# uniio/ivf-hnsw

Hardware: AMD Instinct MI355X
Metric: queries/sec @ Recall@1, SIFT1B PQ16 nprobe=32; ADC scan HBM GB/s vs peak (higher is better)
Workload: dtype f32

## Files before the change

ivf-hnsw_amd/csrc/capi_handle.cpp:

```cpp
#include "capi_internal.h"

#include <cstdarg>

static thread_local std::string g_last_error;

namespace ivfhnsw_gpu_impl {

int fail(int code, const char *fmt, ...)
{
    char buf[512];
    va_list ap;
    va_start(ap, fmt);
    vsnprintf(buf, sizeof(buf), fmt, ap);
    va_end(ap);
    g_last_error = buf;
    return code;
}

int bind(ivfhnsw_gpu *h)
{
    if (!h)
        return fail(IVFHNSW_ERR_INVALID, "null handle");
    HIP_TRY(hipSetDevice(h->device));
    return IVFHNSW_OK;
// ... 18 lines not shown
    }
    hipEvent_t e = nullptr;
    (void)hipEventCreate(&e);
    return e;
}

int drain_events(ivfhnsw_gpu *h)
{
    for (auto &ev : h->pending) {
        HIP_TRY(hipEventSynchronize(ev.b));
        float ms = 0.f;
        HIP_TRY(hipEventElapsedTime(&ms, ev.a, ev.b));
        h->stage_ms[ev.stage] += ms;
        h->stage_n[ev.stage] += 1;
        h->pool.push_back(ev.a);
        h->pool.push_back(ev.b);
    }
    h->pending.clear();
    return IVFHNSW_OK;
}

int check_status(ivfhnsw_gpu *h)
{
    uint32_t st = 0;
    HIP_TRY(hipMemcpy(&st, &status_words(h)->bits, sizeof(st), hipMemcpyDeviceToHost));
    if (!st)
        return IVFHNSW_OK;
    HIP_TRY(hipMemset(&status_words(h)->bits, 0, sizeof(st)));
    if (st & kStatusHnswTieOverflow)
        return fail(IVFHNSW_ERR_STATE, "HNSW walk: more than 64 candidates tie exactly with the efSearch-th "
                                       "distance; results of this batch are invalid");
    if (st & kStatusTopkStreamOverflow)
        return fail(IVFHNSW_ERR_STATE, "heap-order top-k: candidate stream of a query exceeded %u entries; use "
                                       "heap_order = 0 for this k / max_codes", kHeapStreamCap);
    return fail(IVFHNSW_ERR_STATE, "device status 0x%x", st);
}

void follow_parent(ivfhnsw_gpu *view, const ivfhnsw_gpu *parent)
{
    view->t = parent->t;
    view->has_ivf = parent->has_ivf;
    view->n_local = parent->n_local;
    view->g = parent->g;
    view->has_group = parent->has_group;
    view->gr = parent->gr;
    view->has_graph = parent->has_graph;
    view->filter_mode = parent->filter_mode;
    view->fmask = parent->fmask;
    view->f_pass = parent->f_pass;
}

int table_change_guard(ivfhnsw_gpu *h, TableChange what, const char *who, bool need_ivf)
{
    if (h && h->is_view) {
        static const char *const kinds[] = {"uploads", "appends", "removals"};
        return fail(IVFHNSW_ERR_STATE, "%s%s%s go to the handle that holds the tables, not to a view of it",
                    what == kUploads ? "" : who, what == kUploads ? "" : ": ", kinds[what]);
    }
    int rc = bind(h);
    if (rc)
        return rc;
    if (need_ivf && !h->has_ivf)
        return fail(IVFHNSW_ERR_STATE, "%s before upload_ivf", who);
    return IVFHNSW_OK;
}

void point_at_lists(ivfhnsw_gpu *h, uint64_t n_local)
{
    h->t.goff = h->goff.as<uint64_t>();
    h->t.loff = h->loff.as<uint32_t>();
    h->t.codes = h->codes.as<uint8_t>();
    h->t.norm_codes = h->ncodes.as<uint8_t>();
    h->t.ids = h->ids.as<uint32_t>();
    h->n_local = n_local;
}

}

const char *ivfhnsw_gpu_last_error(void) { return g_last_error.c_str(); }

int ivfhnsw_gpu_abi_version(void) { return 9; }

int ivfhnsw_gpu_device_count(int *count)
{
    if (!count)
        return fail(IVFHNSW_ERR_INVALID, "null argument");
    int n = 0;
    hipError_t e = hipGetDeviceCount(&n);
    if (e != hipSuccess)
        return fail(IVFHNSW_ERR_HIP, "hipGetDeviceCount: %s", hipGetErrorString(e));
    *count = n;
    return IVFHNSW_OK;
}

static int split_permille_env()
{
    static const int v = [] {
        const char *e = getenv("IVFHNSW_SPLIT");
        const int x = (e && *e) ? atoi(e) : kSplitAuto;
        return (x > 0 && x <= kSplitAuto) ? x : 0;
    }();
    return v;
}

int ivfhnsw_gpu_create(int device, ivfhnsw_gpu **out)
{
    if (!out)
        return fail(IVFHNSW_ERR_INVALID, "null out pointer");
    *out = nullptr;
    int ndev = 0;
    hipError_t e = hipGetDeviceCount(&ndev);
    if (e != hipSuccess || ndev == 0)
        return fail(IVFHNSW_ERR_HIP, "no HIP device available (%s); there is no CPU fallback",
                    e == hipSuccess ? "device count 0" : hipGetErrorString(e));
    if (device < 0 || device >= ndev)
        return fail(IVFHNSW_ERR_INVALID, "device %d out of range (have %d)", device, ndev);
    HIP_TRY(hipSetDevice(device));
    hipDeviceProp_t prop;
    HIP_TRY(hipGetDeviceProperties(&prop, device));
    if (strncmp(prop.gcnArchName, "gfx950", 6) != 0)
        return fail(IVFHNSW_ERR_HIP, "device %d is %s; this library holds gfx950 code only", device, prop.gcnArchName);
    ivfhnsw_gpu *h = new ivfhnsw_gpu();
    h->device = device;
    hipError_t se = hipStreamCreateWithFlags(&h->stream, hipStreamNonBlocking);
    if (se != hipSuccess) {
        delete h;
        return fail(IVFHNSW_ERR_HIP, "hipStreamCreate: %s", hipGetErrorString(se));
    }
    h->own_stream = true;
    h->split_pm = split_permille_env();
    if (h->w_status.ensure(sizeof(StatusWords)) || hipMemset(h->w_status.p, 0, sizeof(StatusWords)) != hipSuccess) {
        ivfhnsw_gpu_destroy(h);
        return fail(IVFHNSW_ERR_HIP, "cannot allocate the device status word");
    }
    *out = h;
    return IVFHNSW_OK;
}

int ivfhnsw_gpu_destroy(ivfhnsw_gpu *h)
{
    if (!h)
        return IVFHNSW_OK;
    (void)hipSetDevice(h->device);
    (void)hipStreamSynchronize(h->stream);
    if (h->split_view) {
        ivfhnsw_gpu_destroy(h->split_view);
        h->split_view = nullptr;
        (void)hipSetDevice(h->device);
    }
    if (h->split_fork)
        (void)hipEventDestroy(h->split_fork);
    if (h->split_join)
        (void)hipEventDestroy(h->split_join);
    for (auto &ev : h->pending) {
        (void)hipEventDestroy(ev.a);
        (void)hipEventDestroy(ev.b);
    }
    for (auto e : h->pool)
        (void)hipEventDestroy(e);
    h->for_each_devbuf([](DevBuf &b) { b.release(); });
    h->p_in.release();
    h->p_out.release();
    if (h->own_stream)
        (void)hipStreamDestroy(h->stream);
    delete h;
    return IVFHNSW_OK;
}

int ivfhnsw_gpu_create_view(ivfhnsw_gpu *parent, ivfhnsw_gpu **out)
{
    if (!out)
        return fail(IVFHNSW_ERR_INVALID, "null out pointer");
    *out = nullptr;
    int rc = bind(parent);
    if (rc)
        return rc;
    if (parent->is_view)
        return fail(IVFHNSW_ERR_INVALID, "a view of a view: create it from the handle that holds the tables");
    HIP_TRY(hipStreamSynchronize(parent->stream));
    ivfhnsw_gpu *h = nullptr;
    if ((rc = ivfhnsw_gpu_create(parent->device, &h)))
        return rc;
    h->is_view = true;
    h->split_pm = 0;
    follow_parent(h, parent);
    h->parent = parent;
    *out = h;
    return IVFHNSW_OK;
}

int ivfhnsw_gpu_set_stream(ivfhnsw_gpu *h, void *hip_stream)
{
    int rc = bind(h);
    if (rc)
        return rc;
    HIP_TRY(hipStreamSynchronize(h->stream));
    if (h->own_stream)
        (void)hipStreamDestroy(h->stream);
    h->stream = reinterpret_cast<hipStream_t>(hip_stream);
    h->own_stream = false;
    return IVFHNSW_OK;
}

int ivfhnsw_gpu_sync(ivfhnsw_gpu *h)
{
    int rc = bind(h);
    if (rc)
        return rc;
    HIP_TRY(hipStreamSynchronize(h->stream));
    return check_status(h);
}

int ivfhnsw_gpu_set_batch_split(ivfhnsw_gpu *h, int permille)
{
    if (!h)
        return fail(IVFHNSW_ERR_INVALID, "null handle");
    if (permille < 0 || permille > kSplitAuto)
        return fail(IVFHNSW_ERR_INVALID, "batch split %d outside 0..999 permille (1000 = by estimate)", permille);
    if (h->is_view && permille)
        return fail(IVFHNSW_ERR_INVALID, "a view cannot split its batches (it is what the second part runs on)");
    h->split_pm = permille;
    return IVFHNSW_OK;
}

int ivfhnsw_gpu_set_option(ivfhnsw_gpu *h, const char *key, long value)
{
    if (!h || !key)
        return fail(IVFHNSW_ERR_INVALID, "set_option: null argument");
    if (!strcmp(key, "scan_pipe")) {
        if (value < -1 || value > 1)
            return fail(IVFHNSW_ERR_INVALID, "set_option scan_pipe: %ld outside -1..1", value);
        h->opt_scan_pipe = (int)value;
        return IVFHNSW_OK;
    }
    if (!strcmp(key, "exact_splits")) {
        if (value != -1 && (value < 1 || value > 64))
            return fail(IVFHNSW_ERR_INVALID, "set_option exact_splits: %ld is neither -1 nor in 1..64", value);
        h->opt_exact_splits = (int)value;
        return IVFHNSW_OK;
    }
    return fail(IVFHNSW_ERR_INVALID, "set_option: unknown key '%s'", key);
}

int ivfhnsw_gpu_set_profiling(ivfhnsw_gpu *h, int enabled)
{
    int rc = bind(h);
    if (rc)
        return rc;
    h->profiling = enabled == 2 ? 2 : (enabled != 0 ? 1 : 0);
    if (h->split_view)
        h->split_view->profiling = h->profiling;
    return IVFHNSW_OK;
}

int ivfhnsw_gpu_get_stage_ms(ivfhnsw_gpu *h, int stage, double *ms_total, uint64_t *launches)
{
    int rc = bind(h);
    if (rc)
        return rc;
    if (stage < 0 || stage >= IVFHNSW_STAGE_COUNT)
        return fail(IVFHNSW_ERR_INVALID, "bad stage %d", stage);
    if ((rc = drain_events(h)))
        return rc;
    double ms = h->stage_ms[stage];
    uint64_t n = h->stage_n[stage];
    if (h->split_view) {
        if ((rc = drain_events(h->split_view)))
            return rc;
        ms += h->split_view->stage_ms[stage];
        n += h->split_view->stage_n[stage];
    }
    if (ms_total)
        *ms_total = ms;
    if (launches)
        *launches = n;
    return IVFHNSW_OK;
}

int ivfhnsw_gpu_reset_stage_ms(ivfhnsw_gpu *h)
{
    int rc = bind(h);
    if (rc)
        return rc;
    if ((rc = drain_events(h)))
        return rc;
    for (int i = 0; i < IVFHNSW_STAGE_COUNT; i++) {
        h->stage_ms[i] = 0;
        h->stage_n[i] = 0;
    }
    if (h->split_view)
        return ivfhnsw_gpu_reset_stage_ms(h->split_view);
    return IVFHNSW_OK;
}

int ivfhnsw_gpu_last_scan_counts(ivfhnsw_gpu *h, uint64_t *ncodes, uint64_t *nsegments)
{
    int rc = bind(h);
    if (rc)
        return rc;
    unsigned long long out[2] = {0, 0};
    if (h->last_nq) {
        HIP_TRY(launch_plan_totals(h->stream, h->w_hdr.as<PlanHdr>(), h->last_nq,
                                   h->w_totals.as<unsigned long long>()));
        HIP_TRY(hipMemcpyAsync(out, h->w_totals.p, sizeof(out), hipMemcpyDeviceToHost, h->stream));
        HIP_TRY(hipStreamSynchronize(h->stream));
    }
// ... 38 lines not shown
```

ivf-hnsw_amd/csrc/capi_internal.h:

```cpp
#pragma once
#include "../../include/ivfhnsw_hip.h"
#include "ivfhnsw_kernels.h"

#include <hip/hip_runtime.h>

#include <algorithm>
#include <new>
#include <cmath>
#include <cstddef>
#include <cstdio>
#include <cstdlib>
#include <cstring>
#include <string>
#include <unordered_map>
#include <vector>

namespace ivfhnsw_gpu_impl {

int fail(int code, const char *fmt, ...) __attribute__((format(printf, 2, 3)));

#define HIP_TRY(expr)                                                                                        \
    do {                                                                                                     \
        hipError_t e_ = (expr);                                                                              \
        if (e_ != hipSuccess)                                                                                \
            return fail(e_ == hipErrorOutOfMemory ? IVFHNSW_ERR_NOMEM : IVFHNSW_ERR_HIP, "%s: %s (%s:%d)",   \
                        #expr, hipGetErrorString(e_), __FILE__, __LINE__);                                   \
    } while (0)

struct DevBuf {
    void *p = nullptr;
    size_t bytes = 0;
    int ensure(size_t need)
    {
        if (need <= bytes)
            return IVFHNSW_OK;
        release();
        HIP_TRY(hipMalloc(&p, need ? need : 1));
        bytes = need;
        return IVFHNSW_OK;
    }
    void release()
    {
        if (p)
            (void)hipFree(p);
        p = nullptr;
        bytes = 0;
    }
    template <class T> T *as() const { return reinterpret_cast<T *>(p); }
};

struct HostBuf {
    void *p = nullptr;
    size_t bytes = 0;
    int ensure(size_t need)
    {
        if (need <= bytes)
            return IVFHNSW_OK;
        release();
        HIP_TRY(hipHostMalloc(&p, need ? need : 1, hipHostMallocDefault));
        bytes = need;
        return IVFHNSW_OK;
    }
    void release()
    {
        if (p)
            (void)hipHostFree(p);
        p = nullptr;
        bytes = 0;
    }
    template <class T> T *as() const { return reinterpret_cast<T *>(p); }
};

struct StageEvent {
    int stage;
    hipEvent_t a, b;
};

struct StatusWords {
    uint32_t bits;
    uint32_t walk_next;
    uint32_t redo_len;
    uint32_t redo_next;
    uint32_t redo_exits;
    uint32_t heap_redo_len;
    uint32_t heap_redo_exits;
    uint32_t pad;
};
static_assert(offsetof(StatusWords, redo_len) == offsetof(StatusWords, walk_next) + 4 &&
                  offsetof(StatusWords, redo_next) == offsetof(StatusWords, walk_next) + 8 &&
                  offsetof(StatusWords, redo_exits) == offsetof(StatusWords, walk_next) + 12,
              "launch_coarse: next_query is followed by the three words of the redo header");
static_assert(offsetof(StatusWords, heap_redo_exits) == offsetof(StatusWords, heap_redo_len) + 4, "launch_heap_scan: redo_hdr[0..1]");
static_assert(offsetof(StatusWords, bits) == 0 && sizeof(StatusWords) == 8 * sizeof(uint32_t), "8 words, bits first");

struct WalkScratch {
    bool zero = false;
    void *zero_ptr = nullptr;
    size_t zero_bytes = 0;
    bool counters_clean = true;
};

}

using namespace ivfhnsw_gpu_impl;

#define IVFHNSW_GPU_DEVBUFS(X) \
    X(goff) X(loff) X(cnorm) X(pqc) X(ntab) X(opq_at) X(codes) X(ncodes) X(ids)  \
    X(g_alpha) X(g_nn) X(g_sizes) X(g_inter)  \
    X(q_counts) X(q_links) X(q_vectors) X(q_qrows) X(q_nbrows) X(q_nbnorms) X(q_fat) X(q_links_c)  \
    X(e_pqc) X(e_ntab) X(e_a) X(e_at) X(e_x) X(e_idx) X(e_dist) X(e_res) X(e_tmp) X(e_codes) X(e_ncodes)  \
    X(t_x) X(t_y) X(t_cb) X(t_assign) X(t_part) X(t_c)  \
    X(k_q) X(k_x) X(k_qn) X(k_xn) X(k_part) X(k_ids) X(k_dists)  \
    X(km_x) X(km_c) X(km_assign) X(km_dist) X(km_cnt) X(km_start) X(km_ids) X(km_ids2) X(km_hist) X(km_part) X(km_status) X(km_pairs)  \
    X(gb_table) X(gb_fwd) X(gb_fcnt) X(gb_deg) X(gb_roff) X(gb_ids) X(gb_ids2) X(gb_hist) X(gb_stat) X(gb_counts) X(gb_links)  \
    X(cg_q) X(cg_cidx) X(cg_ids) X(cg_dists) X(gc_nn) X(cg_cvn) X(cg_tab) X(cg_tab2) X(cg_off) X(cg_alpha2) X(cg_sub)  \
    X(base_rows) X(base_stage)  \
    X(r_q) X(r_cand) X(r_dist) X(r_lab)  \
    X(ex_q) X(ex_part) X(ex_raw) X(ex_dist) X(ex_lab)  \
    X(ap_idx) X(ap_ids) X(ap_codes) X(ap_ncodes) X(ap_cnt) X(ap_own) X(ap_part) X(ap_status) X(ap_perm) X(ap_perm2) X(ap_hist) X(ap_tiles)  \
    X(gp_sub) X(gp_sizes) X(gp_pre_old) X(gp_pre_new) X(gp_rows) X(gp_gather) X(ga_cidx) X(ga_off) X(ga_nn) X(ga_alpha) X(ga_inter) X(ga_status)  \
    X(rm_labels) X(rm_bits) X(rm_mask) X(rm_keep) X(rm_rem) X(rm_out) X(rm_part) X(rm_status) X(rm_sizes)  \
    X(f_mask) X(f_bits) X(f_labels) X(f_count)  \
    X(w_xq) X(w_luts) X(w_segs) X(w_lpos) X(w_hdr) X(w_keys) X(w_cid) X(w_cd) X(w_qsd) X(w_totals) X(w_visited) X(w_status) X(w_stream) X(w_slen) X(w_tail) X(w_redo) X(w_hredo) X(w_heap)  \
    X(rg_dist) X(rg_lab) X(rg_slices) X(rg_part) X(rg_lims)  \
    X(s_q) X(s_cid) X(s_cd) X(s_dist) X(s_lab) X(s_keys) X(s_len)

struct ivfhnsw_gpu {
    int device = 0;
    hipStream_t stream = nullptr;
    bool own_stream = false;
    bool is_view = false;

#define IVFHNSW_X(name) DevBuf name;
    IVFHNSW_GPU_DEVBUFS(IVFHNSW_X)
#undef IVFHNSW_X
    template <class F> void for_each_devbuf(F &&f)
    {
#define IVFHNSW_X(name) f(name);
        IVFHNSW_GPU_DEVBUFS(IVFHNSW_X)
#undef IVFHNSW_X
    }
    HostBuf p_in, p_out;

    IvfTables t{};
    bool has_ivf = false;
    uint64_t n_local = 0;
    GroupTables g{};
    bool has_group = false;
    GraphTables gr{};
    bool has_graph = false;
    size_t e_d = 0, e_M = 0;
    bool e_opq = false, has_codebooks = false;
    uint64_t base_n = 0;
    size_t base_d = 0;
    ivfhnsw_gpu *parent = nullptr;

    int filter_mode = -1;
    const uint32_t *fmask = nullptr;
    bool f_has_bits = false;
    uint32_t f_max_label = 0;
    uint64_t f_pass = 0;

    ivfhnsw_gpu *split_view = nullptr;
    hipEvent_t split_fork = nullptr, split_join = nullptr;
    bool last_split = false;
    uint32_t *status_shared = nullptr;
    size_t last_parts[2] = {0, 0};
    int split_pm = 0;
    WalkScratch walk;
    int opt_scan_pipe = -1;
    int opt_exact_splits = -1;

    int last_nq = 0, last_max_seg = 0;
    const char *last_scan_kernel = "";
    bool last_stream = false;
    bool last_range = false;

    bool rg_valid = false;
    uint64_t rg_total = 0;

    int profiling = 0;
    std::vector<StageEvent> pending;
    std::vector<hipEvent_t> pool;
    double stage_ms[IVFHNSW_STAGE_COUNT] = {0};
    uint64_t stage_n[IVFHNSW_STAGE_COUNT] = {0};
};

namespace ivfhnsw_gpu_impl {

int bind(ivfhnsw_gpu *h);
int upload(DevBuf &b, const void *src, size_t bytes);
hipEvent_t take_event(ivfhnsw_gpu *h);
int drain_events(ivfhnsw_gpu *h);
int check_status(ivfhnsw_gpu *h);

inline StatusWords *status_words(ivfhnsw_gpu *h) { return h->w_status.as<StatusWords>(); }
inline uint32_t *status_word(ivfhnsw_gpu *h) { return h->status_shared ? h->status_shared : &status_words(h)->bits; }

void follow_parent(ivfhnsw_gpu *view, const ivfhnsw_gpu *parent);

enum TableChange { kUploads, kAppends, kRemovals };
int table_change_guard(ivfhnsw_gpu *h, TableChange what, const char *who, bool need_ivf);

void point_at_lists(ivfhnsw_gpu *h, uint64_t n_local);

int filter_mark_rows(ivfhnsw_gpu *h, const uint32_t *ids, uint64_t n_local, DevBuf &mask, uint64_t *pass);
void filter_drop(ivfhnsw_gpu *h);

struct ListArrays {
    DevBuf goff, loff, codes, ncodes, ids;
    DevBuf fmask;
    uint64_t fpass = 0;
    ListArrays() = default;
    ListArrays(const ListArrays &) = delete;
    ListArrays &operator=(const ListArrays &) = delete;
    ~ListArrays() { release(); }
    int allocate(size_t nc, uint64_t n_local, size_t M)
    {
        int rc;
        if ((rc = goff.ensure((nc + 1) * sizeof(uint64_t))) || (rc = loff.ensure(nc * sizeof(uint32_t))) ||
            (rc = codes.ensure(n_local * M)) || (rc = ncodes.ensure(n_local)) || (rc = ids.ensure(n_local * sizeof(uint32_t))))
            return rc;
        return IVFHNSW_OK;
    }
    int mark_filter(ivfhnsw_gpu *h, uint64_t n_local)
    {
        if (h->filter_mode < 0)
            return IVFHNSW_OK;
        return filter_mark_rows(h, ids.as<uint32_t>(), n_local, fmask, &fpass);
    }
    void release()
    {
        for (DevBuf *b : {&goff, &loff, &codes, &ncodes, &ids, &fmask})
            b->release();
    }
    void install(ivfhnsw_gpu *h, uint64_t n_local)
    {
        if (h->filter_mode >= 0) {
            std::swap(h->f_mask, fmask);
            h->fmask = h->f_mask.as<uint32_t>();
            h->f_pass = fpass;
        }
        std::swap(h->goff, goff);
        std::swap(h->loff, loff);
        std::swap(h->codes, codes);
        std::swap(h->ncodes, ncodes);
        std::swap(h->ids, ids);
        release();
        point_at_lists(h, n_local);
    }
};

struct StageScope {
    ivfhnsw_gpu *h;
    StageEvent ev{};
    bool on;
    StageScope(ivfhnsw_gpu *h_, int stage)
        : h(h_), on(h_->profiling == 1 || (h_->profiling == 2 && stage == IVFHNSW_STAGE_SCAN))
    {
        if (!on)
            return;
        ev.stage = stage;
        ev.a = take_event(h);
        ev.b = take_event(h);
        (void)hipEventRecord(ev.a, h->stream);
    }
    ~StageScope()
    {
        if (!on)
            return;
        (void)hipEventRecord(ev.b, h->stream);
        h->pending.push_back(ev);
    }
};

constexpr uint32_t kHeapStreamCap = 8192;

constexpr int kSplitAuto = 1000;

constexpr size_t kMaxBatchAll = 1 << 17;

struct SearchCall {
    uint32_t *status_out = nullptr;
    bool defer_redo = false;
    bool no_latency = false;
    bool wrote_status = false;
};

struct WalkClear {
    uint64_t *keys = nullptr;
    uint32_t *done = nullptr;
    bool cleared = false;
};

struct SearchArgs {
    size_t nq, k;
    const float *d_queries;
    const uint32_t *d_coarse_ids;
    const float *d_coarse_dists;
    const ivfhnsw_search_params *p;
    float *d_distances;
    int64_t *d_labels, *d_out_keys;
    SearchArgs slice(size_t q0, size_t n, size_t d) const
    {
        return {n, k, d_queries + q0 * d, d_coarse_ids ? d_coarse_ids + q0 * p->nprobe : nullptr,
                d_coarse_dists ? d_coarse_dists + q0 * p->nprobe : nullptr, p, d_distances + q0 * k, d_labels + q0 * k,
                d_out_keys};
    }
};

struct Chunk : SearchArgs {
    int nprobe, max_seg, plan_k;
    bool heap_big;
    const uint32_t *fmask;
    const float *xq;
    const uint32_t *cid;
    const float *cd;
    bool use_tail;
    WalkClear meet;
    int nsplit;
    bool heap, pipe;
};

int search_args_guard(const ivfhnsw_gpu *h, const ivfhnsw_search_params *p, size_t k);
int stage_in(ivfhnsw_gpu *h, DevBuf &b, const void *src, size_t bytes);
int stage_out(ivfhnsw_gpu *h, void *dst, const DevBuf &b, size_t bytes);
int chunk_checks(ivfhnsw_gpu *h, const Chunk &c, bool results = true);
int chunk_workspace(ivfhnsw_gpu *h, Chunk &c);
int chunk_coarse(ivfhnsw_gpu *h, Chunk &c, const SearchCall &call);
int chunk_plan_table(ivfhnsw_gpu *h, Chunk &c);

void range_drop(ivfhnsw_gpu *h);

int grouping_dedupe_reserve(ivfhnsw_gpu *h);
int grouping_dedupe_dev(ivfhnsw_gpu *h, const uint32_t *d_sizes, const uint32_t *d_nn, int *dedupe);

int encode_rows(ivfhnsw_gpu *h, size_t m, float *dx, const float *table, const uint32_t *rows);
int encode_groups_impl(ivfhnsw_gpu *h, size_t ngroups, size_t nsubc, const uint32_t *centroid_idx,
                       const uint64_t *offsets, const float *x, size_t efSearch, uint32_t *out_nn_centroid_idxs,
                       float *out_alphas, uint32_t *out_subcentroid_idxs, uint8_t *out_codes, uint8_t *out_norm_codes,
                       bool dev, bool stage);

}
```

ivf-hnsw_amd/csrc/capi_search.cpp:

```cpp
#include "capi_internal.h"

static size_t env_size(const char *name, size_t def)
{
    const char *e = getenv(name);
    return (e && *e) ? (size_t)atol(e) : def;
}

int ivfhnsw_gpu_impl::search_args_guard(const ivfhnsw_gpu *h, const ivfhnsw_search_params *p, size_t k)
{
    if (!h->has_ivf)
        return fail(IVFHNSW_ERR_STATE, "search before upload_ivf");
    if (!p || p->nprobe == 0 || k == 0)
        return fail(IVFHNSW_ERR_INVALID, "nprobe and k must be positive");
    return IVFHNSW_OK;
}

int ivfhnsw_gpu_impl::stage_in(ivfhnsw_gpu *h, DevBuf &b, const void *src, size_t bytes)
{
    int rc = b.ensure(bytes);
    if (rc)
        return rc;
    HIP_TRY(hipMemcpyAsync(b.p, src, bytes, hipMemcpyHostToDevice, h->stream));
    return IVFHNSW_OK;
}

int ivfhnsw_gpu_impl::stage_out(ivfhnsw_gpu *h, void *dst, const DevBuf &b, size_t bytes)
{
    HIP_TRY(hipMemcpyAsync(dst, b.p, bytes, hipMemcpyDeviceToHost, h->stream));
    return IVFHNSW_OK;
}

static int walk_scratch(ivfhnsw_gpu *h, size_t words, size_t nslots, size_t nq, uint32_t **tails)
{
    int rc = h->w_visited.ensure(words * sizeof(uint32_t) * std::max<size_t>(nslots, 64) * 2);
    if (rc)
        return rc;
    if (h->w_visited.p != h->walk.zero_ptr || h->w_visited.bytes != h->walk.zero_bytes) {
        HIP_TRY(hipMemsetAsync(h->w_visited.p, 0, h->w_visited.bytes, h->stream));
        h->walk.zero = true;
        h->walk.zero_ptr = h->w_visited.p;
        h->walk.zero_bytes = h->w_visited.bytes;
    }
    *tails = reinterpret_cast<uint32_t *>(h->w_visited.as<char>() + h->w_visited.bytes / 2);
    return h->w_redo.ensure(nq * sizeof(uint32_t));
}

static int coarse_dev_impl(ivfhnsw_gpu *h, size_t nq, const float *d_queries, size_t nprobe, size_t efSearch,
                           uint32_t *d_coarse_ids, float *d_coarse_dists, const SearchCall &call, WalkClear &meet)
{
    int rc = bind(h);
    if (rc)
        return rc;
    if (!h->has_graph)
        return fail(IVFHNSW_ERR_STATE, "coarse search needs upload_quantizer");
    if (nprobe == 0 || efSearch < nprobe)
        return fail(IVFHNSW_ERR_INVALID, "efSearch %zu < nprobe %zu (precondition of IndexIVF_HNSW.cpp:249-258)",
                    efSearch, nprobe);
    if (efSearch > 1024)
        return fail(IVFHNSW_ERR_INVALID, "efSearch %zu > 1024 unsupported on the device", efSearch);
    if (nq == 0)
        return IVFHNSW_OK;
    if (nq > 0x7fffffffull)
        return fail(IVFHNSW_ERR_INVALID, "nq too large");
    const size_t words = ((((size_t)h->gr.n + 31) / 32) + 3) & ~(size_t)3;
    StageScope sc(h, IVFHNSW_STAGE_COARSE);
    static const size_t lat_max_nq = env_size("IVFHNSW_LATENCY_MAX_NQ", 256);
    StatusWords *st = status_words(h);
    uint32_t *tails = nullptr;
    if (!call.no_latency && nq <= lat_max_nq && coarse_latency_supported(h->gr, (int)efSearch)) {
        uint32_t *hdr = &st->redo_len;
        const bool defer = call.defer_redo;
        if (!defer) {
            if ((rc = walk_scratch(h, words, 64, nq, &tails)))
                return rc;
            HIP_TRY(hipMemsetAsync(hdr, 0, 3 * sizeof(uint32_t), h->stream));
        }
        HIP_TRY(launch_coarse_latency(h->stream, h->gr, d_queries, (int)nq, (int)nprobe, (int)efSearch, d_coarse_ids,
                                      d_coarse_dists, status_word(h), meet.keys, meet.done, defer ? nullptr : hdr,
                                      defer ? nullptr : h->w_redo.as<uint32_t>()));
        meet.cleared = meet.keys != nullptr;
        if (!defer)
            HIP_TRY(launch_coarse_redo(h->stream, h->gr, d_queries, (int)nq, (int)nprobe, (int)efSearch, d_coarse_ids,
                                       d_coarse_dists, h->w_visited.as<uint32_t>(), words, status_word(h), hdr,
                                       h->w_redo.as<uint32_t>(), tails, 64));
        return IVFHNSW_OK;
    }
    const int nslots = (int)std::min<size_t>(nq, (size_t)coarse_slots_for((int)efSearch));
    if ((rc = walk_scratch(h, words, (size_t)nslots, nq, &tails)))
        return rc;
    HIP_TRY(launch_coarse(h->stream, h->gr, d_queries, (int)nq, (int)nprobe, (int)efSearch, d_coarse_ids, d_coarse_dists,
                          h->w_visited.as<uint32_t>(), words, nslots, status_word(h), &st->walk_next,
                          h->w_visited.bytes / 2, &h->walk.zero, h->w_redo.as<uint32_t>(), tails, 64,
                          &h->walk.counters_clean));
    return IVFHNSW_OK;
}

int ivfhnsw_gpu_coarse_dev(ivfhnsw_gpu *h, size_t nq, const float *d_queries, size_t nprobe, size_t efSearch,
                           uint32_t *d_coarse_ids, float *d_coarse_dists)
{
    WalkClear meet;
    return coarse_dev_impl(h, nq, d_queries, nprobe, efSearch, d_coarse_ids, d_coarse_dists, SearchCall(), meet);
}

int ivfhnsw_gpu_rotate_dev(ivfhnsw_gpu *h, size_t nq, const float *d_queries, float *d_out)
{
    int rc = bind(h);
    if (rc)
        return rc;
    if (!h->has_ivf)
        return fail(IVFHNSW_ERR_STATE, "rotate needs upload_ivf");
    if (nq == 0)
        return IVFHNSW_OK;
    if (!d_queries || !d_out || nq > 0x7fffffffull)
        return fail(IVFHNSW_ERR_INVALID, "null buffer or nq too large");
    if (h->t.opq_At) {
        StageScope sc(h, IVFHNSW_STAGE_OPQ);
        HIP_TRY(launch_opq(h->stream, h->t.opq_At, d_queries, d_out, (int)nq, h->t.d));
    } else if (d_out != d_queries) {
        HIP_TRY(hipMemcpyAsync(d_out, d_queries, nq * (size_t)h->t.d * sizeof(float), hipMemcpyDeviceToDevice, h->stream));
    }
    return IVFHNSW_OK;
}

int ivfhnsw_gpu_coarse(ivfhnsw_gpu *h, size_t nq, const float *queries, size_t k, size_t efSearch, uint32_t *ids,
                       float *dists)
{
    int rc = bind(h);
    if (rc)
        return rc;
    if (!h->has_graph)
        return fail(IVFHNSW_ERR_STATE, "coarse search needs upload_quantizer");
    if (nq == 0)
        return IVFHNSW_OK;
    if (!queries || !ids || !dists || k == 0)
        return fail(IVFHNSW_ERR_INVALID, "null buffer or k == 0");
    const size_t d = h->gr.d;
    if ((rc = h->s_cid.ensure(nq * k * sizeof(uint32_t))) || (rc = h->s_cd.ensure(nq * k * sizeof(float))) ||
        (rc = stage_in(h, h->s_q, queries, nq * d * sizeof(float))) ||
        (rc = ivfhnsw_gpu_coarse_dev(h, nq, h->s_q.as<float>(), k, efSearch, h->s_cid.as<uint32_t>(), h->s_cd.as<float>())) ||
        (rc = stage_out(h, ids, h->s_cid, nq * k * sizeof(uint32_t))) ||
        (rc = stage_out(h, dists, h->s_cd, nq * k * sizeof(float))))
        return rc;
    HIP_TRY(hipStreamSynchronize(h->stream));
    return check_status(h);
}

static int search_dev_chunk(ivfhnsw_gpu *h, const SearchArgs &a, SearchCall &call);

static const size_t kSplitMinNq = 8192;

static int auto_split_permille(const ivfhnsw_gpu *h, const ivfhnsw_search_params *p)
{
    const double walk = 1.7 * (double)p->efSearch;
    const double nc = (double)std::max<uint32_t>(h->t.nc, 1u);
    const double list = (double)h->n_local / nc;
    const double codes = std::min((double)p->nprobe * list, (double)p->max_codes + 0.5 * list);
    double scan = codes * (double)(h->t.M + 1) / 5000.0 + 5.0;
    if (h->has_group)
        scan = scan / 0.8 + 90.0;
    const double share = walk / (walk + scan);
    return (int)std::min(900.0, std::max(400.0, share * 1000.0 + 0.5));
}

static int search_dev_split(ivfhnsw_gpu *h, const SearchArgs &a, SearchCall &call)
{
    const size_t nq = a.nq;
    int rc = bind(h);
    if (rc)
        return rc;
    if (!h->split_view) {
        if ((rc = ivfhnsw_gpu_create_view(h, &h->split_view)))
            return rc;
        HIP_TRY(hipEventCreateWithFlags(&h->split_fork, hipEventDisableTiming));
        HIP_TRY(hipEventCreateWithFlags(&h->split_join, hipEventDisableTiming));
    }
    ivfhnsw_gpu *v = h->split_view;
    follow_parent(v, h);
    v->profiling = h->profiling;
    v->status_shared = &status_words(h)->bits;
    const size_t round_wgs = 2048;
    const int pm = h->split_pm == kSplitAuto ? auto_split_permille(h, a.p) : h->split_pm;
    size_t n2 = ((nq * (size_t)(1000 - pm) / 1000 + round_wgs / 2) / round_wgs) * round_wgs;
    n2 = std::max(round_wgs, std::min(n2, nq / 2));
    const size_t n1 = nq - n2;
    HIP_TRY(hipEventRecord(h->split_fork, h->stream));
    HIP_TRY(hipStreamWaitEvent(v->stream, h->split_fork, 0));
    rc = search_dev_chunk(h, a.slice(0, n1, (size_t)h->t.d), call);
    int rc2 = rc ? rc : search_dev_chunk(v, a.slice(n1, n2, (size_t)h->t.d), call);
    (void)hipSetDevice(h->device);
    HIP_TRY(hipEventRecord(h->split_join, v->stream));
    HIP_TRY(hipStreamWaitEvent(h->stream, h->split_join, 0));
    h->last_split = rc2 == 0;
    h->last_parts[0] = n1;
    h->last_parts[1] = n2;
    return rc2;
}

static int search_dev_part(ivfhnsw_gpu *h, const SearchArgs &a, SearchCall &call)
{
    if (h) {
        h->last_split = false;
        h->last_parts[0] = a.nq;
        h->last_parts[1] = 0;
    }
    const bool split = h && a.p && !h->is_view && h->split_pm > 0 && a.nq >= kSplitMinNq && !a.d_coarse_ids &&
                       !a.d_out_keys && !(a.p->heap_order && a.k > 1) && h->has_ivf && h->has_graph && a.p->nprobe > 0 &&
                       a.k > 0 && a.k <= 1024 && a.d_queries && a.d_distances && a.d_labels;
    return split ? search_dev_split(h, a, call) : search_dev_chunk(h, a, call);
}

static int search_dev_impl(ivfhnsw_gpu *h, const SearchArgs &a, SearchCall &call)
{
    const size_t kMaxBatch = (a.p && a.p->heap_order && a.k > 1) ? kMaxBatchAll / 8 : kMaxBatchAll;
    if (a.nq <= kMaxBatch || !h || !a.p)
        return search_dev_part(h, a, call);
    if (a.d_out_keys)
        return fail(IVFHNSW_ERR_INVALID, "sharded search (out_keys) is limited to %zu queries per call", kMaxBatch);
    for (size_t q0 = 0; q0 < a.nq; q0 += kMaxBatch) {
        int rc = search_dev_part(h, a.slice(q0, std::min(kMaxBatch, a.nq - q0), (size_t)h->t.d), call);
        if (rc)
            return rc;
    }
    return IVFHNSW_OK;
}

int ivfhnsw_gpu_search_dev(ivfhnsw_gpu *h, size_t nq, size_t k, const float *d_queries, const uint32_t *d_coarse_ids,
                           const float *d_coarse_dists, const ivfhnsw_search_params *p, float *d_distances,
                           int64_t *d_labels, int64_t *d_out_keys)
{
    SearchCall call;
    return search_dev_impl(h, {nq, k, d_queries, d_coarse_ids, d_coarse_dists, p, d_distances, d_labels, d_out_keys}, call);
}

static void remember_plan(ivfhnsw_gpu *h, size_t nq, int max_seg, bool has_stream, const char *kernel_name)
{
    h->last_scan_kernel = kernel_name;
    h->last_nq = (int)nq;
    h->last_max_seg = max_seg;
    h->last_stream = has_stream;
}

int ivfhnsw_gpu_impl::chunk_checks(ivfhnsw_gpu *h, const Chunk &c, bool results)
{
    int rc = bind(h);
    if (rc || (rc = search_args_guard(h, c.p, c.k)))
        return rc;
    if ((c.d_coarse_ids == nullptr) != (c.d_coarse_dists == nullptr))
        return fail(IVFHNSW_ERR_INVALID, "coarse_ids and coarse_dists must both be given or both be NULL");
    if (c.nq > 0 && (!c.d_queries || (results && (!c.d_distances || !c.d_labels))))
        return fail(IVFHNSW_ERR_INVALID, "null query/result buffer");
    if (c.k > 1024 && (!c.p->heap_order || c.d_out_keys))
        return fail(IVFHNSW_ERR_INVALID, "k %zu > 1024 unsupported (only heap_order = 1 without out_keys)", c.k);
    if (c.nq > 0x7fffffffull / (c.k > c.p->nprobe ? c.k : c.p->nprobe))
        return fail(IVFHNSW_ERR_INVALID, "nq too large");
    if (h->has_group && !h->has_graph)
        return fail(IVFHNSW_ERR_STATE, "Grouping search needs upload_quantizer (sub-centroid distances)");
    if (h->has_graph && (h->gr.d != h->t.d || h->gr.n != h->t.nc))
        return fail(IVFHNSW_ERR_STATE, "quantizer (%u x %d) does not match the index (%u x %d)", h->gr.n, h->gr.d,
                    h->t.nc, h->t.d);
    return IVFHNSW_OK;
}

int ivfhnsw_gpu_impl::chunk_workspace(ivfhnsw_gpu *h, Chunk &c)
{
    c.nprobe = (int)c.p->nprobe;
    c.max_seg = h->has_group ? c.nprobe * h->g.nsubc : c.nprobe;
    c.heap_big = c.k > 1024;
    c.plan_k = c.heap_big ? 1 : (int)c.k;
    c.fmask = h->filter_mode >= 0 ? h->fmask : nullptr;
    int rc;
    if ((rc = h->w_segs.ensure(c.nq * (size_t)c.max_seg * sizeof(Seg))) ||
        (rc = h->w_lpos.ensure(c.nq * (size_t)c.max_seg * sizeof(uint32_t))) ||
        (rc = h->w_hdr.ensure(c.nq * sizeof(PlanHdr))) ||
        (rc = h->w_keys.ensure(c.nq * (size_t)c.plan_k * sizeof(uint64_t))) ||
        (rc = h->w_totals.ensure(2 * sizeof(unsigned long long))))
        return rc;
    return IVFHNSW_OK;
}

int ivfhnsw_gpu_impl::chunk_coarse(ivfhnsw_gpu *h, Chunk &c, const SearchCall &call)
{
    const size_t nq = c.nq;
    int rc;
    c.xq = c.d_queries;
    if (h->t.opq_At) {
        if ((rc = h->w_xq.ensure(nq * (size_t)h->t.d * sizeof(float))))
            return rc;
        StageScope sc(h, IVFHNSW_STAGE_OPQ);
        HIP_TRY(launch_opq(h->stream, h->t.opq_At, c.d_queries, h->w_xq.as<float>(), (int)nq, h->t.d));
        c.xq = h->w_xq.as<float>();
    }
    static const size_t tail_max_nq = env_size("IVFHNSW_TAIL_MAX_NQ", 8);
    c.use_tail = !h->has_group && nq <= tail_max_nq && !c.d_out_keys && !c.fmask &&
                 ivf_tail_supported(h->t, c.nprobe, (int)c.k);
    if (c.use_tail) {
        if ((rc = h->w_tail.ensure(nq * (sizeof(uint64_t) + sizeof(uint32_t)))))
            return rc;
        c.meet.keys = h->w_tail.as<uint64_t>();
        c.meet.done = reinterpret_cast<uint32_t *>(c.meet.keys + nq);
    }
    c.cid = c.d_coarse_ids;
    c.cd = c.d_coarse_dists;
    if (!c.cid) {
        if ((rc = h->w_cid.ensure(nq * (size_t)c.nprobe * sizeof(uint32_t))) ||
            (rc = h->w_cd.ensure(nq * (size_t)c.nprobe * sizeof(float))) ||
            (rc = coarse_dev_impl(h, nq, c.xq, c.p->nprobe, c.p->efSearch, h->w_cid.as<uint32_t>(), h->w_cd.as<float>(),
                                  call, c.meet)))
            return rc;
        c.cid = h->w_cid.as<uint32_t>();
        c.cd = h->w_cd.as<float>();
    }
    return IVFHNSW_OK;
}

static int chunk_tail(ivfhnsw_gpu *h, const Chunk &c, SearchCall &call)
{
    const size_t nq = c.nq;
    const int nsplit = (int)std::min<size_t>(32, (2048 + nq - 1) / nq);
    StageScope sc(h, IVFHNSW_STAGE_SCAN);
    if (!c.meet.cleared)
        HIP_TRY(hipMemsetAsync(c.meet.keys, 0, nq * (sizeof(uint64_t) + sizeof(uint32_t)), h->stream));
    HIP_TRY(launch_ivf_tail(h->stream, h->t, c.xq, c.cid, c.cd, (int)nq, c.nprobe, c.p->max_codes, nsplit, c.meet.keys,
                            c.meet.done, h->w_hdr.as<PlanHdr>(), c.d_distances, c.d_labels, status_word(h),
                            call.status_out));
    call.wrote_status = call.status_out != nullptr;
    remember_plan(h, nq, c.max_seg, false, "ivf_tail_kernel");
    return IVFHNSW_OK;
}

int ivfhnsw_gpu_impl::chunk_plan_table(ivfhnsw_gpu *h, Chunk &c)
{
    const int nq = (int)c.nq, max_seg = c.max_seg;
    const ivfhnsw_search_params *p = c.p;
    int rc;
    c.heap = p->heap_order && c.k > 1;
    c.nsplit = (c.k == 1 && c.nq < 1024) ? (int)std::min<size_t>(32, (2048 + c.nq - 1) / c.nq) : 1;
    c.pipe = c.k == 1 && !h->has_group && !c.heap && !c.fmask && h->opt_scan_pipe != 0 &&
             scan_pipe_supported(h->t, max_seg, nq, c.nsplit, h->n_local > 0, h->opt_scan_pipe == 1);
    static const bool plan_lut_on = env_size("IVFHNSW_PLAN_LUT", 1) != 0;
    const int ds = h->t.dsub;
    const bool plan_lut = plan_lut_on && !h->has_group && !c.pipe && h->t.shard_world == 1 &&
                          (ds == 4 || ds == 6 || ds == 8 || ds == 12 || ds == 16);
    if (!c.pipe && (rc = h->w_luts.ensure(c.nq * (size_t)h->t.M * 256 * sizeof(float))))
        return rc;
    Seg *segs = h->w_segs.as<Seg>();
    uint32_t *lpos = h->w_lpos.as<uint32_t>();
    PlanHdr *hdr = h->w_hdr.as<PlanHdr>();
    uint64_t *keys = h->w_keys.as<uint64_t>();
    if (plan_lut) {
        StageScope sc(h, IVFHNSW_STAGE_LUT);
        HIP_TRY(launch_plan_lut(h->stream, h->t, c.xq, c.cid, c.cd, nq, c.nprobe, p->max_codes, segs, lpos, hdr, max_seg,
                                keys, c.plan_k, h->w_luts.as<float>()));
        return IVFHNSW_OK;
    }
    {
        StageScope sc(h, IVFHNSW_STAGE_PLAN);
        if (h->has_group) {
            if ((rc = h->w_qsd.ensure(c.nq * (size_t)max_seg * 2 * sizeof(float))))
                return rc;
            HIP_TRY(launch_plan_grouping(h->stream, h->t, h->g, h->gr, c.xq, c.cid, c.cd, nq, c.nprobe, p->max_codes,
                                         p->do_pruning, segs, lpos, hdr, max_seg, keys, c.plan_k, h->w_qsd.as<float>()));
        } else {
            HIP_TRY(launch_plan_ivf(h->stream, h->t, c.cid, c.cd, nq, c.nprobe, p->max_codes, segs, lpos, hdr, max_seg,
                                    keys, c.plan_k));
        }
    }
    if (!c.pipe) {
        StageScope sc(h, IVFHNSW_STAGE_LUT);
        HIP_TRY(launch_lut(h->stream, h->t, c.xq, h->w_luts.as<float>(), nq, hdr));
    }
    return IVFHNSW_OK;
}

static int chunk_scan_select(ivfhnsw_gpu *h, const Chunk &c)
{
    const int nq = (int)c.nq, k = (int)c.k, max_seg = c.max_seg;
    const bool heap = c.heap, replay_here = c.heap && !c.d_out_keys;
    float *luts = h->w_luts.as<float>();
    Seg *segs = h->w_segs.as<Seg>();
    uint32_t *lpos = h->w_lpos.as<uint32_t>();
    PlanHdr *hdr = h->w_hdr.as<PlanHdr>();
    int rc;
    float *heap_ws = nullptr;
    if (replay_here) {
        if ((rc = h->w_heap.ensure(heap_scan_ws_bytes(h->t.M, k, nq))))
            return rc;
        heap_ws = h->w_heap.as<float>();
    }
    if (c.heap_big) {
        {
            StageScope sc(h, IVFHNSW_STAGE_SCAN);
            HIP_TRY(launch_heap_scan(h->stream, h->t, luts, segs, lpos, hdr, max_seg, nq, k, nullptr, nullptr, heap_ws,
                                     c.d_distances, c.d_labels, c.fmask));
        }
        remember_plan(h, c.nq, max_seg, false, c.fmask ? "heap_scan_kernel+filter" : "heap_scan_kernel");
        return IVFHNSW_OK;
    }
    if (heap) {
        if ((rc = h->w_stream.ensure(c.nq * (size_t)kHeapStreamCap * sizeof(uint64_t))) ||
            (rc = h->w_slen.ensure(c.nq * sizeof(uint32_t))) ||
            (replay_here && (rc = h->w_hredo.ensure(c.nq * sizeof(uint32_t)))))
            return rc;
    }
    bool scan_selected = false;
    const char *kernel_name = "scan_pipe_kernel";
    {
        StageScope sc(h, IVFHNSW_STAGE_SCAN);
        if (c.pipe) {
            HIP_TRY(launch_scan_pipe(h->stream, h->t, c.xq, segs, lpos, hdr, max_seg, nq, h->w_keys.as<uint64_t>()));
        } else {
            const uint64_t nseg_all = (uint64_t)h->t.nc * (h->has_group ? (uint64_t)h->g.nsubc : 1);
            const int seg_hint =
                (int)std::min<uint64_t>(1u << 20, nseg_all ? (h->n_local * h->t.shard_world) / nseg_all : 0);
            const bool want_sel = k == 1 && !c.d_out_keys && !heap;
            HIP_TRY(launch_scan(h->stream, h->t, luts, segs, lpos, hdr, max_seg, nq, k, c.nsplit, h->w_keys.as<uint64_t>(),
                                heap ? h->w_stream.as<uint64_t>() : nullptr, heap ? h->w_slen.as<uint32_t>() : nullptr,
                                heap ? kHeapStreamCap : 0, seg_hint, want_sel ? c.d_distances : nullptr,
                                want_sel ? c.d_labels : nullptr, &scan_selected, c.fmask));
            kernel_name = last_scan_kernel_name();
        }
    }
    if (!scan_selected) {
        StageScope sc(h, IVFHNSW_STAGE_SELECT);
        if (replay_here) {
            uint32_t *redo_hdr = &status_words(h)->heap_redo_len;
            HIP_TRY(launch_heap_replay(h->stream, h->t, segs, hdr, max_seg, h->w_stream.as<uint64_t>(),
                                       h->w_slen.as<uint32_t>(), kHeapStreamCap, nq, k, c.d_distances, c.d_labels,
                                       status_word(h), nullptr, redo_hdr, h->w_hredo.as<uint32_t>()));
            HIP_TRY(launch_heap_scan(h->stream, h->t, luts, segs, lpos, hdr, max_seg, nq, k, redo_hdr,
                                     h->w_hredo.as<uint32_t>(), heap_ws, c.d_distances, c.d_labels, c.fmask));
        } else
            HIP_TRY(launch_select(h->stream, h->t, segs, hdr, max_seg, h->w_keys.as<uint64_t>(), nq, k, c.d_distances,
                                  c.d_labels, c.d_out_keys));
    }
    remember_plan(h, c.nq, max_seg, heap, kernel_name);
    return IVFHNSW_OK;
}

static int search_dev_chunk(ivfhnsw_gpu *h, const SearchArgs &a, SearchCall &call)
{
    Chunk c{a};
    int rc = chunk_checks(h, c);
    if (rc)
        return rc;
    h->last_nq = 0;
    h->last_range = false;
    call.wrote_status = false;
    if (c.nq == 0)
        return IVFHNSW_OK;
    if ((rc = chunk_workspace(h, c)) || (rc = chunk_coarse(h, c, call)))
        return rc;
    if (c.use_tail)
        return chunk_tail(h, c, call);
    if ((rc = chunk_plan_table(h, c)))
        return rc;
    return chunk_scan_select(h, c);
}

int ivfhnsw_gpu_resolve_keys_dev(ivfhnsw_gpu *h, size_t nq, size_t k, const int64_t *d_keys, float *d_distances,
                                 int64_t *d_labels)
{
    int rc = bind(h);
    if (rc)
        return rc;
    if (!h->has_ivf || h->last_nq == 0 || (size_t)h->last_nq != nq || h->last_range)
        return fail(IVFHNSW_ERR_STATE, "resolve_keys needs the plan of a preceding search_dev with the same nq");
    StageScope sc(h, IVFHNSW_STAGE_SELECT);
    HIP_TRY(launch_resolve(h->stream, h->t, h->w_segs.as<Seg>(), h->w_hdr.as<PlanHdr>(), h->last_max_seg, d_keys,
                           (int)nq, (int)k, d_distances, d_labels));
    return IVFHNSW_OK;
}

int ivfhnsw_gpu_last_stream_dev(ivfhnsw_gpu *h, size_t nq, size_t len_cap, uint64_t *d_keys, uint32_t *d_len,
                                uint32_t *stream_cap)
{
    int rc = bind(h);
    if (rc)
        return rc;
    if (!h->last_nq || !h->last_stream || (size_t)h->last_nq != nq)
        return fail(IVFHNSW_ERR_STATE, "last_stream needs a preceding search_dev of the same nq with k > 1 and heap_order = 1");
    if (stream_cap)
        *stream_cap = kHeapStreamCap;
    if (d_len)
        HIP_TRY(hipMemcpyAsync(d_len, h->w_slen.p, nq * sizeof(uint32_t), hipMemcpyDeviceToDevice, h->stream));
    if (d_keys) {
        if (len_cap == 0 || len_cap > kHeapStreamCap)
            return fail(IVFHNSW_ERR_INVALID, "len_cap %zu outside 1..%u", len_cap, kHeapStreamCap);
        HIP_TRY(hipMemcpy2DAsync(d_keys, len_cap * sizeof(uint64_t), h->w_stream.p, (size_t)kHeapStreamCap * sizeof(uint64_t),
                                 len_cap * sizeof(uint64_t), nq, hipMemcpyDeviceToDevice, h->stream));
    }
    return IVFHNSW_OK;
}

int ivfhnsw_gpu_replay_stream_dev(ivfhnsw_gpu *h, size_t nq, size_t k, const uint64_t *d_stream, const uint32_t *d_len,
                                  uint32_t cap, int64_t *d_out_keys)
{
    int rc = bind(h);
    if (rc)
        return rc;
    if (!h->has_ivf)
        return fail(IVFHNSW_ERR_STATE, "replay_stream before upload_ivf");
    if (nq == 0)
        return IVFHNSW_OK;
    if (!d_stream || !d_len || !d_out_keys || k == 0 || k > 1024 || nq > 0x7fffffffull / k)
        return fail(IVFHNSW_ERR_INVALID, "bad replay_stream arguments (k %zu)", k);
    StageScope sc(h, IVFHNSW_STAGE_SELECT);
    HIP_TRY(launch_heap_replay(h->stream, h->t, nullptr, nullptr, 0, d_stream, d_len, cap, (int)nq, (int)k, nullptr,
                               nullptr, status_word(h), d_out_keys));
    return IVFHNSW_OK;
}

int ivfhnsw_gpu_search(ivfhnsw_gpu *h, size_t nq, size_t k, const float *queries, const uint32_t *coarse_ids,
                       const float *coarse_dists, const ivfhnsw_search_params *p, float *distances, int64_t *labels)
{
    int rc = bind(h);
    if (rc || (rc = search_args_guard(h, p, k)))
        return rc;
    if (nq == 0)
        return IVFHNSW_OK;
    if (!queries || !distances || !labels)
        return fail(IVFHNSW_ERR_INVALID, "null query/result buffer");
    if ((coarse_ids == nullptr) != (coarse_dists == nullptr))
        return fail(IVFHNSW_ERR_INVALID, "coarse_ids and coarse_dists must both be given or both be NULL");
    const size_t in_q = nq * h->t.d * sizeof(float), in_c = coarse_ids ? nq * p->nprobe * sizeof(uint32_t) : 0;
    static const size_t pinned_max_nq = env_size("IVFHNSW_PINNED_MAX_NQ", 256);
    if (nq <= pinned_max_nq) {
        const size_t out_d = (nq * k * sizeof(float) + 7) & ~(size_t)7, out_l = nq * k * sizeof(int64_t);
        if ((rc = h->p_in.ensure(in_q + 2 * in_c)) || (rc = h->p_out.ensure(out_d + out_l + 8)))
            return rc;
        char *pin = h->p_in.as<char>(), *pout = h->p_out.as<char>();
        memcpy(pin, queries, in_q);
        if (coarse_ids) {
            memcpy(pin + in_q, coarse_ids, in_c);
            memcpy(pin + in_q + in_c, coarse_dists, in_c);
        }
        uint32_t *pst = reinterpret_cast<uint32_t *>(pout + out_d + out_l);
        uint32_t *bits = &status_words(h)->bits;
        for (int attempt = 0; attempt < 2; attempt++) {
            SearchCall call{pst, attempt == 0, attempt == 1};
            rc = search_dev_impl(h,
                                 {nq, k, reinterpret_cast<const float *>(pin),
                                  coarse_ids ? reinterpret_cast<const uint32_t *>(pin + in_q) : nullptr,
                                  coarse_ids ? reinterpret_cast<const float *>(pin + in_q + in_c) : nullptr, p,
                                  reinterpret_cast<float *>(pout), reinterpret_cast<int64_t *>(pout + out_d), nullptr},
                                 call);
            if (rc)
                return rc;
            if (!call.wrote_status)
                HIP_TRY(hipMemcpyAsync(pst, bits, sizeof(uint32_t), hipMemcpyDeviceToHost, h->stream));
            HIP_TRY(hipStreamSynchronize(h->stream));
            if (attempt == 0 && (*pst & kStatusHnswTieOverflow)) {
                *pst &= ~kStatusHnswTieOverflow;
                HIP_TRY(hipMemcpy(bits, pst, sizeof(uint32_t), hipMemcpyHostToDevice));
                continue;
            }
            break;
        }
        memcpy(distances, pout, nq * k * sizeof(float));
        memcpy(labels, pout + out_d, out_l);
        return *pst ? check_status(h) : IVFHNSW_OK;
    }
    if ((rc = h->s_dist.ensure(nq * k * sizeof(float))) || (rc = h->s_lab.ensure(nq * k * sizeof(int64_t))) ||
        (rc = stage_in(h, h->s_q, queries, in_q)) ||
        (coarse_ids && ((rc = stage_in(h, h->s_cid, coarse_ids, in_c)) || (rc = stage_in(h, h->s_cd, coarse_dists, in_c)))) ||
        (rc = ivfhnsw_gpu_search_dev(h, nq, k, h->s_q.as<float>(), coarse_ids ? h->s_cid.as<uint32_t>() : nullptr,
                                     coarse_ids ? h->s_cd.as<float>() : nullptr, p, h->s_dist.as<float>(),
                                     h->s_lab.as<int64_t>(), nullptr)) ||
        (rc = stage_out(h, distances, h->s_dist, nq * k * sizeof(float))) ||
        (rc = stage_out(h, labels, h->s_lab, nq * k * sizeof(int64_t))))
        return rc;
    HIP_TRY(hipStreamSynchronize(h->stream));
    return check_status(h);
}

int ivfhnsw_gpu_search_keys(ivfhnsw_gpu *h, size_t nq, size_t k, const float *queries, const uint32_t *coarse_ids,
                            const float *coarse_dists, const ivfhnsw_search_params *p, int64_t *keys)
{
    int rc = bind(h);
    if (rc || (rc = search_args_guard(h, p, k)))
        return rc;
    if (nq == 0)
        return IVFHNSW_OK;
    if (!queries || !keys || !coarse_ids || !coarse_dists)
        return fail(IVFHNSW_ERR_INVALID, "null buffer (a shard is searched with the coarse stage supplied)");
    const size_t d = h->t.d, np = p->nprobe;
    if ((rc = h->s_dist.ensure(nq * k * sizeof(float))) || (rc = h->s_lab.ensure(nq * k * sizeof(int64_t))) ||
        (rc = h->s_keys.ensure(nq * k * sizeof(int64_t))) || (rc = stage_in(h, h->s_q, queries, nq * d * sizeof(float))) ||
        (rc = stage_in(h, h->s_cid, coarse_ids, nq * np * sizeof(uint32_t))) ||
        (rc = stage_in(h, h->s_cd, coarse_dists, nq * np * sizeof(float))) ||
        (rc = ivfhnsw_gpu_search_dev(h, nq, k, h->s_q.as<float>(), h->s_cid.as<uint32_t>(), h->s_cd.as<float>(), p,
                                     h->s_dist.as<float>(), h->s_lab.as<int64_t>(), h->s_keys.as<int64_t>())) ||
        (rc = stage_out(h, keys, h->s_keys, nq * k * sizeof(int64_t))))
        return rc;
    HIP_TRY(hipStreamSynchronize(h->stream));
    return check_status(h);
}

int ivfhnsw_gpu_resolve_keys(ivfhnsw_gpu *h, size_t nq, size_t k, const int64_t *keys, float *distances, int64_t *labels)
{
    int rc = bind(h);
    if (rc)
        return rc;
// ... 31 lines not shown
```

Baseline: 6.082 million.

## Build PQ lookup tables early on a low-priority side stream during split search

In split search, the per-query ADC lookup tables are now computed on a separate low-priority stream as soon as the queries are ready, while the coarse HNSW walk runs on the main stream. The plan and scan then wait on an event for those tables. This stops LUT construction from serialising behind the coarse walk. The auto split ratio is also retuned to drop the fixed LUT cost from the scan estimate. In exchange it adds an extra stream, events and cross-stream dependencies, and the side stream competes with the walk for compute units.

```diff
diff --git a/ivf-hnsw_amd/csrc/capi_handle.cpp b/ivf-hnsw_amd/csrc/capi_handle.cpp
--- a/ivf-hnsw_amd/csrc/capi_handle.cpp
+++ b/ivf-hnsw_amd/csrc/capi_handle.cpp
@@ -194,6 +194,13 @@
         (void)hipEventDestroy(h->split_fork);
     if (h->split_join)
         (void)hipEventDestroy(h->split_join);
+    if (h->early_stream) {
+        (void)hipStreamSynchronize(h->early_stream);
+        (void)hipStreamDestroy(h->early_stream);
+    }
+    for (hipEvent_t e : {h->early_ready[0], h->early_ready[1], h->early_done[0], h->early_done[1]})
+        if (e)
+            (void)hipEventDestroy(e);
     for (auto &ev : h->pending) {
         (void)hipEventDestroy(ev.a);
         (void)hipEventDestroy(ev.b);
diff --git a/ivf-hnsw_amd/csrc/capi_internal.h b/ivf-hnsw_amd/csrc/capi_internal.h
--- a/ivf-hnsw_amd/csrc/capi_internal.h
+++ b/ivf-hnsw_amd/csrc/capi_internal.h
@@ -163,6 +163,10 @@
 
     ivfhnsw_gpu *split_view = nullptr;
     hipEvent_t split_fork = nullptr, split_join = nullptr;
+    hipStream_t early_stream = nullptr;
+    hipEvent_t early_ready[2] = {nullptr, nullptr};
+    hipEvent_t early_done[2] = {nullptr, nullptr};
+    bool early_failed = false;
     bool last_split = false;
     uint32_t *status_shared = nullptr;
     size_t last_parts[2] = {0, 0};
@@ -253,23 +257,24 @@
 
 struct StageScope {
     ivfhnsw_gpu *h;
+    hipStream_t s;
     StageEvent ev{};
     bool on;
-    StageScope(ivfhnsw_gpu *h_, int stage)
-        : h(h_), on(h_->profiling == 1 || (h_->profiling == 2 && stage == IVFHNSW_STAGE_SCAN))
+    StageScope(ivfhnsw_gpu *h_, int stage, hipStream_t s_ = nullptr)
+        : h(h_), s(s_ ? s_ : h_->stream), on(h_->profiling == 1 || (h_->profiling == 2 && stage == IVFHNSW_STAGE_SCAN))
     {
         if (!on)
             return;
         ev.stage = stage;
         ev.a = take_event(h);
         ev.b = take_event(h);
-        (void)hipEventRecord(ev.a, h->stream);
+        (void)hipEventRecord(ev.a, s);
     }
     ~StageScope()
     {
         if (!on)
             return;
-        (void)hipEventRecord(ev.b, h->stream);
+        (void)hipEventRecord(ev.b, s);
         h->pending.push_back(ev);
     }
 };
@@ -279,12 +284,19 @@
 constexpr int kSplitAuto = 1000;
 
 constexpr size_t kMaxBatchAll = 1 << 17;
+
+struct EarlyTables {
+    hipStream_t stream;
+    hipEvent_t ready;
+    hipEvent_t done;
+};
 
 struct SearchCall {
     uint32_t *status_out = nullptr;
     bool defer_redo = false;
     bool no_latency = false;
     bool wrote_status = false;
+    const EarlyTables *early = nullptr;
 };
 
 struct WalkClear {
@@ -320,6 +332,7 @@
     WalkClear meet;
     int nsplit;
     bool heap, pipe;
+    const EarlyTables *early;
 };
 
 int search_args_guard(const ivfhnsw_gpu *h, const ivfhnsw_search_params *p, size_t k);
diff --git a/ivf-hnsw_amd/csrc/capi_search.cpp b/ivf-hnsw_amd/csrc/capi_search.cpp
--- a/ivf-hnsw_amd/csrc/capi_search.cpp
+++ b/ivf-hnsw_amd/csrc/capi_search.cpp
@@ -147,19 +147,60 @@
 
 static int search_dev_chunk(ivfhnsw_gpu *h, const SearchArgs &a, SearchCall &call);
 
+static bool plan_lut_shape(const ivfhnsw_gpu *h)
+{
+    static const bool plan_lut_on = env_size("IVFHNSW_PLAN_LUT", 1) != 0;
+    const int ds = h->t.dsub;
+    return plan_lut_on && !h->has_group && h->t.shard_world == 1 && (ds == 4 || ds == 6 || ds == 8 || ds == 12 || ds == 16);
+}
+
 static const size_t kSplitMinNq = 8192;
 
-static int auto_split_permille(const ivfhnsw_gpu *h, const ivfhnsw_search_params *p)
+static int auto_split_permille(const ivfhnsw_gpu *h, const ivfhnsw_search_params *p, bool early_tables)
 {
     const double walk = 1.7 * (double)p->efSearch;
     const double nc = (double)std::max<uint32_t>(h->t.nc, 1u);
     const double list = (double)h->n_local / nc;
     const double codes = std::min((double)p->nprobe * list, (double)p->max_codes + 0.5 * list);
-    double scan = codes * (double)(h->t.M + 1) / 5000.0 + 5.0;
+    double scan = codes * (double)(h->t.M + 1) / 5000.0 + (early_tables ? 0.0 : 5.0);
     if (h->has_group)
         scan = scan / 0.8 + 90.0;
     const double share = walk / (walk + scan);
     return (int)std::min(900.0, std::max(400.0, share * 1000.0 + 0.5));
+}
+
+static bool early_tables_wanted(const ivfhnsw_gpu *h, const SearchArgs &a)
+{
+    static const bool on = env_size("IVFHNSW_EARLY_LUT", 1) != 0;
+    if (!on || !plan_lut_shape(h) || h->filter_mode >= 0)
+        return false;
+    const bool may_pipe = a.k == 1 && h->opt_scan_pipe != 0 &&
+                          scan_pipe_supported(h->t, (int)a.p->nprobe, (int)a.nq, 1, h->n_local > 0, h->opt_scan_pipe == 1);
+    return !may_pipe;
+}
+
+static bool early_setup(ivfhnsw_gpu *h)
+{
+    if (h->early_stream)
+        return true;
+    if (h->early_failed)
+        return false;
+    int least = 0, greatest = 0;
+    hipStream_t s = nullptr;
+    bool ok = hipDeviceGetStreamPriorityRange(&least, &greatest) == hipSuccess &&
+              hipStreamCreateWithPriority(&s, hipStreamNonBlocking, least) == hipSuccess;
+    for (int i = 0; i < 2 && ok; i++)
+        ok = hipEventCreateWithFlags(&h->early_ready[i], hipEventDisableTiming) == hipSuccess &&
+             hipEventCreateWithFlags(&h->early_done[i], hipEventDisableTiming) == hipSuccess;
+    if (!ok) {
+        (void)hipGetLastError();
+        if (s)
+            (void)hipStreamDestroy(s);
+        h->early_failed = true;
+        return false;
+    }
+    h->early_stream = s;
+    return true;
 }
 
 static int search_dev_split(ivfhnsw_gpu *h, const SearchArgs &a, SearchCall &call)
@@ -179,15 +220,32 @@
     v->profiling = h->profiling;
     v->status_shared = &status_words(h)->bits;
     const size_t round_wgs = 2048;
-    const int pm = h->split_pm == kSplitAuto ? auto_split_permille(h, a.p) : h->split_pm;
-    size_t n2 = ((nq * (size_t)(1000 - pm) / 1000 + round_wgs / 2) / round_wgs) * round_wgs;
-    n2 = std::max(round_wgs, std::min(n2, nq / 2));
-    const size_t n1 = nq - n2;
+    auto second_part = [&](bool early_tables) {
+        const int pm = h->split_pm == kSplitAuto ? auto_split_permille(h, a.p, early_tables) : h->split_pm;
+        const size_t n = ((nq * (size_t)(1000 - pm) / 1000 + round_wgs / 2) / round_wgs) * round_wgs;
+        return std::max(round_wgs, std::min(n, nq / 2));
+    };
+    const bool early = early_tables_wanted(h, a) && second_part(true) < (size_t)coarse_slots_for((int)a.p->efSearch) &&
+                       early_setup(h);
+    const size_t n2 = second_part(early), n1 = nq - n2;
     HIP_TRY(hipEventRecord(h->split_fork, h->stream));
     HIP_TRY(hipStreamWaitEvent(v->stream, h->split_fork, 0));
+    EarlyTables part[2];
+    if (early) {
+        HIP_TRY(hipStreamWaitEvent(h->early_stream, h->split_fork, 0));
+        for (int i = 0; i < 2; i++)
+            part[i] = {h->early_stream, h->early_ready[i], h->early_done[i]};
+    }
+    call.early = early ? &part[0] : nullptr;
     rc = search_dev_chunk(h, a.slice(0, n1, (size_t)h->t.d), call);
+    call.early = early ? &part[1] : nullptr;
     int rc2 = rc ? rc : search_dev_chunk(v, a.slice(n1, n2, (size_t)h->t.d), call);
+    call.early = nullptr;
     (void)hipSetDevice(h->device);
+    if (early && rc2) {
+        HIP_TRY(hipEventRecord(h->early_done[1], h->early_stream));
+        HIP_TRY(hipStreamWaitEvent(h->stream, h->early_done[1], 0));
+    }
     HIP_TRY(hipEventRecord(h->split_join, v->stream));
     HIP_TRY(hipStreamWaitEvent(h->stream, h->split_join, 0));
     h->last_split = rc2 == 0;
@@ -286,9 +344,15 @@
     if (h->t.opq_At) {
         if ((rc = h->w_xq.ensure(nq * (size_t)h->t.d * sizeof(float))))
             return rc;
-        StageScope sc(h, IVFHNSW_STAGE_OPQ);
-        HIP_TRY(launch_opq(h->stream, h->t.opq_At, c.d_queries, h->w_xq.as<float>(), (int)nq, h->t.d));
+        {
+            StageScope sc(h, IVFHNSW_STAGE_OPQ);
+            HIP_TRY(launch_opq(h->stream, h->t.opq_At, c.d_queries, h->w_xq.as<float>(), (int)nq, h->t.d));
+        }
         c.xq = h->w_xq.as<float>();
+        if (call.early) {
+            HIP_TRY(hipEventRecord(call.early->ready, h->stream));
+            HIP_TRY(hipStreamWaitEvent(call.early->stream, call.early->ready, 0));
+        }
     }
     static const size_t tail_max_nq = env_size("IVFHNSW_TAIL_MAX_NQ", 8);
     c.use_tail = !h->has_group && nq <= tail_max_nq && !c.d_out_keys && !c.fmask &&
@@ -337,16 +401,28 @@
     c.nsplit = (c.k == 1 && c.nq < 1024) ? (int)std::min<size_t>(32, (2048 + c.nq - 1) / c.nq) : 1;
     c.pipe = c.k == 1 && !h->has_group && !c.heap && !c.fmask && h->opt_scan_pipe != 0 &&
              scan_pipe_supported(h->t, max_seg, nq, c.nsplit, h->n_local > 0, h->opt_scan_pipe == 1);
-    static const bool plan_lut_on = env_size("IVFHNSW_PLAN_LUT", 1) != 0;
-    const int ds = h->t.dsub;
-    const bool plan_lut = plan_lut_on && !h->has_group && !c.pipe && h->t.shard_world == 1 &&
-                          (ds == 4 || ds == 6 || ds == 8 || ds == 12 || ds == 16);
+    const bool plan_lut = !c.pipe && plan_lut_shape(h);
     if (!c.pipe && (rc = h->w_luts.ensure(c.nq * (size_t)h->t.M * 256 * sizeof(float))))
         return rc;
     Seg *segs = h->w_segs.as<Seg>();
     uint32_t *lpos = h->w_lpos.as<uint32_t>();
     PlanHdr *hdr = h->w_hdr.as<PlanHdr>();
     uint64_t *keys = h->w_keys.as<uint64_t>();
+    if (plan_lut && c.early) {
+        const EarlyTables &e = *c.early;
+        {
+            StageScope sc(h, IVFHNSW_STAGE_LUT, e.stream);
+            HIP_TRY(launch_lut(e.stream, h->t, c.xq, h->w_luts.as<float>(), nq, nullptr));
+        }
+        HIP_TRY(hipEventRecord(e.done, e.stream));
+        {
+            StageScope sc(h, IVFHNSW_STAGE_PLAN);
+            HIP_TRY(launch_plan_ivf(h->stream, h->t, c.cid, c.cd, nq, c.nprobe, p->max_codes, segs, lpos, hdr, max_seg,
+                                    keys, c.plan_k));
+        }
+        HIP_TRY(hipStreamWaitEvent(h->stream, e.done, 0));
+        return IVFHNSW_OK;
+    }
     if (plan_lut) {
         StageScope sc(h, IVFHNSW_STAGE_LUT);
         HIP_TRY(launch_plan_lut(h->stream, h->t, c.xq, c.cid, c.cd, nq, c.nprobe, p->max_codes, segs, lpos, hdr, max_seg,
@@ -448,6 +524,7 @@
     call.wrote_status = false;
     if (c.nq == 0)
         return IVFHNSW_OK;
+    c.early = call.early;
     if ((rc = chunk_workspace(h, c)) || (rc = chunk_coarse(h, c, call)))
         return rc;
     if (c.use_tail)
```

After: 6.212 million (median of 6 runs). 1.02x the previous value.
